# crisbodnar/text-to-image

Measured on AMD Instinct MI355X. Metric: images/sec (G+D step) at 64x64 batch=64, higher is better.
Workload: dtype f32; 1 GPU; wgancls 64x64 batch=64/GPU fp32, synthetic images + random 1024-d text embeddings, D step (+kt) then G step, Adam(b1=0,b2=0.9); global_batch=64, parallelism=dp1, launch=hipGraph replay (1 graph/iteration)

## Files before the change

### include/t2i_hip.h

```cpp
#ifndef T2I_HIP_H
#define T2I_HIP_H

#include <stddef.h>
#include <stdint.h>

#ifdef __cplusplus
extern "C" {
#endif

#define T2I_OK 0
#define T2I_ERR_INVALID (-1)
#define T2I_ERR_WORKSPACE (-2)
#define T2I_ERR_LAUNCH (-3)

#define T2I_ACT_NONE 0
#define T2I_ACT_LRELU 1
#define T2I_ACT_RELU 2
#define T2I_ACT_TANH 3

typedef void* t2i_stream_t;

enum { T2I_DT_F32 = 0, T2I_DT_BF16 = 1 };

typedef struct t2i_conv_desc {
// ... 79 lines not shown
               t2i_stream_t stream);

size_t t2i_bn_bwd_fused_workspace_bytes(int64_t rows, int32_t C);
int t2i_bn_bwd_fused(const void* dy, const void* y, const void* x, const float* mean, const float* rstd, const float* gamma, int64_t rows,
                     int32_t C, int act, float alpha, void* gmask, void* dx, void* dx_h, float* dgamma, float* dbeta, int accumulate, void* ws,
                     size_t ws_bytes, int32_t dtype , t2i_stream_t stream);

size_t t2i_bn_grouped_workspace_bytes(int64_t rows_per_group, int32_t C, int32_t groups);
int t2i_bn_train_fwd_grouped(const void* x, int64_t rows_per_group, int32_t C, int32_t groups, const float* gamma, const float* beta, float eps,
                             float decay, float* mean, float* rstd, float* scale, float* shift, float* moving_mean, float* moving_var, int act,
                             float alpha, void* y, void* y_h, const float* tile_sum, const float* tile_m2, int32_t tile_chunks, int32_t tile_rows,
                             int32_t moving_updates, int32_t moving_groups, void* ws, size_t ws_bytes, int32_t dtype, t2i_stream_t stream);
int t2i_bn_bwd_grouped(const void* dy, const void* y, const void* x, const float* mean, const float* rstd, const float* gamma, int64_t rows_per_group,
                       int32_t C, int32_t groups, int act, float alpha, void* gmask, void* dx, void* dx_h, float* dgamma, float* dbeta, int accumulate,
                       void* ws, size_t ws_bytes, int32_t dtype, t2i_stream_t stream);

int t2i_act_fwd(const void* x, int64_t n, int act, float alpha, void* y, void* y_h, int32_t dtype, t2i_stream_t stream);
int t2i_act_bwd(const void* dy, const void* y, int64_t n, int act, float alpha, void* dx, void* dx_h, int32_t dtype, t2i_stream_t stream);
int t2i_act_bwd_colsum(const void* dy, const void* y, const void* x2, const float* center, int64_t rows, int32_t C, int act,
                       float alpha, void* dx, void* dx_h, float* colsum, float* colsum_x2, int accumulate, void* ws, size_t ws_bytes,
                       int32_t dtype, t2i_stream_t stream);
int t2i_add_act(const void* a, const void* b, int64_t n, int act, float alpha, void* y, void* y_h, int32_t dtype, t2i_stream_t stream);
int t2i_axpby(const void* a, float alpha, const void* b, float beta, int64_t n, void* y, int32_t dtype, t2i_stream_t stream);
int t2i_interp(const float* eps, const float* g, const float* x, int32_t B, int64_t per_sample, float* xhat,
               t2i_stream_t stream);
int t2i_concat_tile_fwd(const void* feat, const void* emb, int32_t B, int32_t P, int32_t Cf, int32_t Ce,
                        void* out, int32_t dtype, t2i_stream_t stream);
int t2i_concat_tile_bwd(const void* dout, int32_t B, int32_t P, int32_t Cf, int32_t Ce, void* dfeat, void* demb,
                        int32_t dtype, t2i_stream_t stream);
int t2i_nchw_to_nhwc(const void* x, int32_t B, int32_t C, int32_t HW, void* y, int32_t dtype, t2i_stream_t stream);
// ... 189 lines not shown
```

### text-to-image_amd/_lib.py

```python
import ctypes
import os

import torch

_HERE = os.path.dirname(os.path.abspath(__file__))
LIB_PATH = os.environ.get('T2I_HIP_LIB', os.path.join(_HERE, 'lib', 'libt2i_hip.so'))


class ConvDesc(ctypes.Structure):
    _fields_ = [(n, ctypes.c_int32) for n in
                ('B', 'H', 'W', 'Cin', 'Ho', 'Wo', 'Cout', 'KH', 'KW', 'SH', 'SW', 'pad_t', 'pad_l', 'math')]


class ConvOpts(ctypes.Structure):
    _fields_ = [('a_image', ctypes.c_void_p), ('b_image', ctypes.c_void_p), ('out_image', ctypes.c_void_p), ('xform', ctypes.c_void_p),
                ('xform_bytes', ctypes.c_size_t), ('xform_mode', ctypes.c_int32), ('out_image_written', ctypes.c_int32),
                ('xform_kept', ctypes.c_int32), ('in_dtype', ctypes.c_int32), ('out_dtype', ctypes.c_int32), ('xform_valid_rows', ctypes.c_int32), ('xform_plane_rows', ctypes.c_int32), ('reserved', ctypes.c_int32)]


class ImageDesc(ctypes.Structure):
    _fields_ = [('offset', ctypes.c_int64)] + [(n, ctypes.c_int32) for n in
                                               ('height', 'width', 'channels', 'y1', 'y2', 'x1', 'x2', 'reserved')]


# ... 32 lines not shown
    't2i_interp': (ctypes.c_int, [_p, _p, _p, _i32, _i64, _p, _p]),
    't2i_concat_tile_fwd': (ctypes.c_int, [_p, _p, _i32, _i32, _i32, _i32, _p, _i32, _p]),
    't2i_concat_tile_bwd': (ctypes.c_int, [_p, _i32, _i32, _i32, _i32, _p, _p, _i32, _p]),
    't2i_nchw_to_nhwc': (ctypes.c_int, [_p, _i32, _i32, _i32, _p, _i32, _p]),
    't2i_nhwc_to_nchw': (ctypes.c_int, [_p, _i32, _i32, _i32, _p, _i32, _p]),
    't2i_gp_slopes': (ctypes.c_int, [_p, _i32, _i64, _p, _i32, _p]),
    't2i_row_scale': (ctypes.c_int, [_p, _p, _i32, _i64, _p, _i32, _p]),
    't2i_row_scale_div': (ctypes.c_int, [_p, _p, _p, _i32, _i64, _p, _i32, _p]),
    't2i_adam_tf': (ctypes.c_int, [_p, _p, _p, _p, _i64, _f, _p, _f, _f, _f, _f, _p]),
    't2i_adam_tf_ema': (ctypes.c_int, [_p, _p, _p, _p, _p, _i64, _f, _p, _f, _f, _f, _f, _f, _p, _p]),
    't2i_adam_tf_slots': (ctypes.c_int, [_p, _p, _p, _p, _p, _i64, _p, _p, _i32, _f, _p, _f, _f, _f, _f, _f, _p, _p]),
    't2i_wgan_d_head': (ctypes.c_int, [_p, _p, _p, _p, _i32, _f, _p, _p, _p, _p, _p]),
    't2i_bn_grouped_workspace_bytes': (_sz, [_i64, _i32, _i32]),
    't2i_bn_train_fwd_grouped': (ctypes.c_int, [_p, _i64, _i32, _i32, _p, _p, _f, _f, _p, _p, _p, _p, _p, _p, ctypes.c_int, _f, _p, _p, _p, _p, _i32, _i32, _i32, _i32, _p, _sz, _i32, _p]),
    't2i_bn_bwd_grouped': (ctypes.c_int, [_p, _p, _p, _p, _p, _p, _i64, _i32, _i32, ctypes.c_int, _f, _p, _p, _p, _p, _p, ctypes.c_int, _p, _sz, _i32, _p]),
    't2i_sigmoid_ce_head': (ctypes.c_int, [_p, _p, _p, _f, _f, _f, _f, _f, _f, _i32, _p, _p, _p, _p, _p, _p, _p, _p]),
    't2i_ca_kl_fwd': (ctypes.c_int, [_p, _p, _p, _i64, _p, _p, _p]),
    't2i_ca_kl_bwd': (ctypes.c_int, [_p, _p, _p, _p, _p, _i64, _p, _p, _p]),
    't2i_lerp_dev': (ctypes.c_int, [_p, _p, _p, _i32, _i64, _p, _p]),
    't2i_conv2d_algo': (ctypes.c_int, [_p, _i32]),
    't2i_stat': (ctypes.c_longlong, [ctypes.c_char_p]),
    't2i_conv2d_bwd_pair': (ctypes.c_int, [_dp, ctypes.c_int, _p, _p, _p, _op, _p, _p, _p, ctypes.c_int, _op, _p, _sz, _p, _sz, _p]),
    't2i_filter_cache_attach': (ctypes.c_int, [_p, _sz]),
    't2i_filter_cache_enable': (ctypes.c_int, [ctypes.c_int]),
    't2i_tuning_set': (ctypes.c_int, [ctypes.c_char_p, ctypes.c_double]),
    't2i_kt_sgd': (ctypes.c_int, [_p, _p, _f, _f, _p]),
    't2i_zero_ranges': (ctypes.c_int, [_p, _p, _i32, _p]),
    't2i_trunc_normal': (ctypes.c_int, [_p, _i64, ctypes.c_uint64, ctypes.c_uint64, _f, _f, _f, _f, _p]),
    't2i_filter_cache_invalidate': (None, [_p, ctypes.c_size_t]),
    't2i_filter_cache_bytes': (ctypes.c_size_t, []),
# ... 102 lines not shown
```

### text-to-image_amd/autograd.py

```python
import contextlib
import weakref

import torch
from torch.autograd import Function
from torch.autograd.function import once_differentiable

from . import kernels as K

_INPUTS_ONLY = [False]

SINKS = {}
NOTIFY = [None]


def register_sink(param, slot, first_touch=None):
    SINKS[param.data_ptr()] = (weakref.ref(param), slot, first_touch)


def sink_accumulate(ptr):
    e = SINKS.get(ptr)
    if e is None or e[2] is None:
        return True
    return not e[2]()

# ... 105 lines not shown
        ctx.set_materialize_grads(False)
        return K.act_bwd(_c(gy), y, act, alpha)

    @staticmethod
    def backward(ctx, gg):
        if gg is None:
            return None, None, None, None
        (y,) = ctx.saved_tensors
        return ActBwdFn.apply(gg, y, ctx.act, ctx.alpha), None, None, None


def _act_bwd(gy, y, act, alpha):
    return ActBwdFn.apply(gy, y, act, alpha) if act != K.ACT_NONE else _c(gy)


class ColSumFn(Function):

    @staticmethod
    def forward(ctx, a):
        ctx.shape, ctx.dtype = a.shape, a.dtype
        return K.col_reduce(_c(a))[0]

    @staticmethod
    def backward(ctx, g):
        return g.to(ctx.dtype).expand(ctx.shape)


class Conv2dFn(Function):

    @staticmethod
# ... 23 lines not shown


def conv2d_backward(x, w, y, gy, geom_b, act, alpha, has_bias, bias_ref, need, xform=None, xform_plane_rows=0):
    params = not _INPUTS_ONLY[0]
    want_b = has_bias and need[2] and params
    gb = None
    bsink = _sink_of(bias_ref) if want_b else None
    if (want_b and act != K.ACT_NONE and not torch.is_grad_enabled() and gy.shape[-1] % 4 == 0):
        gpre, gb = K.act_bwd_colsum(_c(gy), y, act, alpha, out=bsink)
        if bsink is not None:
            gb = None
            _notify(bias_ref)
    else:
        gpre = _act_bwd(gy, y, act, alpha)
        if want_b and bsink is not None:
            K.col_reduce(_c(gpre), out=bsink)
            _notify(bias_ref)
        elif want_b:
            gb = ColSumFn.apply(gpre)
    if need[0] and need[1] and params and _pair_ok(gpre, x, w):
        gx = K.conv_bwd_pair(K.PAIR_BWD_DATA, _c(gpre), w, _c(x), _c(gpre), geom_b[0], geom_b[1], sink_at(w.data_ptr()), out_dtype=x.dtype,
                             accumulate=sink_accumulate(w.data_ptr()))
        _notify(w)
        return gx, None, gb
    gx = ConvBwdDataFn.apply(gpre, w, None, geom_b, K.ACT_NONE, 0.0, x.dtype) if need[0] else None
    gw = _filter_grad(x, gpre, geom_b, w, xform, xform_plane_rows) if (need[1] and params) else None
    return gx, gw, gb


class ConvBwdDataFn(Function):

    @staticmethod
    def forward(ctx, dy, w, b, geom, act, alpha, out_dtype=None):
        d, ws = geom
# ... 18 lines not shown
def bwd_data_backward(dy, w, out, gg, geom_b, act, alpha, has_bias, bias_ref, need):
    gpre = _act_bwd(gg, out, act, alpha)
    params = not _INPUTS_ONLY[0]
    if need[0] and need[1] and params and _pair_ok(gpre, dy, w):
        g_dy = K.conv_bwd_pair(K.PAIR_FWD, _c(gpre), w, _c(gpre), _c(dy), geom_b[0], geom_b[1], sink_at(w.data_ptr()), out_dtype=dy.dtype,
                               accumulate=sink_accumulate(w.data_ptr()))
        _notify(w)
        g_w = None
    else:
        g_dy = Conv2dFn.apply(gpre, w, None, geom_b, K.ACT_NONE, 0.0, False, dy.dtype) if need[0] else None
        g_w = _filter_grad(gpre, dy, geom_b, w) if (need[1] and params) else None
    g_b = None
    if has_bias and need[2] and params:
        bsink = _sink_of(bias_ref)
        if bsink is not None:
            K.col_reduce(_c(gpre), out=bsink)
            _notify(bias_ref)
        else:
            g_b = ColSumFn.apply(gpre)
    return g_dy, g_w, g_b


class ConvBwdFilterFn(Function):

    @staticmethod
    def forward(ctx, x, dy, geom):
        d, ws = geom
        x, dy = _c(x), _c(dy)
        ctx.save_for_backward(x, dy)
        ctx.geom = geom
        return K.conv_bwd_filter(x, dy, d, ws)

    @staticmethod
    def backward(ctx, ggw):
# ... 112 lines not shown
        if gy is None:
            return (None,) * 10
        x, gamma, mean, rstd, y = ctx.saved_tensors
        gy = _c(gy)
        fused = gy.shape[-1] % 4 == 0 and all(t.data_ptr() % 16 == 0 for t in (gy, x, mean))
        if not fused:
            if ctx.act != K.ACT_NONE:
                gy = K.act_bwd(gy, y, ctx.act, ctx.alpha)
            sum_dy, sum_dy_x = K.col_reduce(gy, x, True, center=mean)
        want_g, want_b = ctx.needs_input_grad[1], ctx.needs_input_grad[2]
        gsink = _sink_of(ctx.gamma_ref) if want_g else None
        bsink = _sink_of(ctx.beta_ref) if want_b else None
        sunk = gsink is not None and bsink is not None
        if fused:
            dx, dgamma, dbeta = K.bn_bwd_grouped(gy, y if ctx.act != K.ACT_NONE else None, x, mean, rstd, gamma, 1, ctx.act, ctx.alpha,
                                                 dgamma_out=gsink if sunk else None, dbeta_out=bsink if sunk else None)
        else:
            dx, dgamma, dbeta = K.bn_bwd(gy, x, mean, rstd, gamma, sum_dy, sum_dy_x, dgamma_out=gsink if sunk else None,
                                         dbeta_out=bsink if sunk else None)
        if sunk:
            _notify(ctx.gamma_ref); _notify(ctx.beta_ref)
            return dx, None, None, None, None, None, None, None, None, None
        return dx, (dgamma if want_g else None), (dbeta if want_b else None), None, None, None, None, None, None, None


class BatchNormTrainGroupedFn(Function):

    @staticmethod
    def _fast(x, groups):
        b = x.shape[0] // groups
        return x.shape[-1] % 4 == 0 and x.data_ptr() % 16 == 0 and (x[:b].numel() * x.element_size()) % 16 == 0
# ... 472 lines not shown
```

### text-to-image_amd/csrc/t2i_aux.hip

```cpp
#include <hip/hip_runtime.h>
#include <stdlib.h>
#include <stdint.h>

#include <type_traits>

#include "t2i_internal.h"

namespace t2i {

static inline int ew_blocks(size_t n_items) {
  size_t b = (n_items + 255) / 256;
  if (b > 2048) b = 2048;
  if (b < 1) b = 1;
  return (int)b;
}

__device__ __forceinline__ float vadd(float a, float b) { return a + b; }
__device__ __forceinline__ float4 vadd(float4 a, float4 b) { return make_float4(a.x + b.x, a.y + b.y, a.z + b.z, a.w + b.w); }
__device__ __forceinline__ float vscale(float a, float s) { return a * s; }
__device__ __forceinline__ float4 vscale(float4 a, float s) { return make_float4(a.x * s, a.y * s, a.z * s, a.w * s); }

__device__ __forceinline__ float vsplat(float s, float) { return s; }
__device__ __forceinline__ float4 vsplat(float s, float4) { return make_float4(s, s, s, s); }

// ... 1013 lines not shown
  const int64_t rbeg = (int64_t)g_own * rows_g + (int64_t)j * rpb;
  int64_t rend = rbeg + rpb;
  if (rend > (int64_t)(g_own + 1) * rows_g) rend = (int64_t)(g_own + 1) * rows_g;
#pragma unroll 4
  for (int64_t r = rbeg + ty; r < rend; r += 16) {
    const size_t e4 = (size_t)(r * C + c) >> 2;
    float4 v = ld4<H>(x, e4);
    v.x = apply_act(v.x * sc.x + sh.x, act, alpha);
    v.y = apply_act(v.y * sc.y + sh.y, act, alpha);
    v.z = apply_act(v.z * sc.z + sh.z, act, alpha);
    v.w = apply_act(v.w * sc.w + sh.w, act, alpha);
    st4(y, yh, e4, v);
  }
}

template <bool HD, bool HX>
__global__ __launch_bounds__(256) void bn_bwd_apply_fused(const float* __restrict__ part0, const float* __restrict__ part1, int nchunks,
                                                          int64_t rows_g, int C, const float* __restrict__ mean, const float* __restrict__ rstd,
                                                          const float* __restrict__ gamma, float* __restrict__ dgamma, float* __restrict__ dbeta,
                                                          int accumulate, int groups, int64_t rpb, int nb_g, const void* __restrict__ gv,
                                                          const void* __restrict__ xv, float* __restrict__ dx, uint2* __restrict__ dxh) {
  __shared__ float4 red[16][16], red1[16][16];
  __shared__ float4 s_a[16], s_b[16], s_e[16];
  const int tx = threadIdx.x & 15, ty = threadIdx.x >> 4;
  const int c = blockIdx.x * 64 + tx * 4;
  const bool col_ok = c < C;
  const int g_own = blockIdx.y / nb_g, j = blockIdx.y - g_own * nb_g;
  const bool scribe = blockIdx.y == 0;
  const float n = (float)rows_g;
  float tg[4] = {0.f, 0.f, 0.f, 0.f}, tb[4] = {0.f, 0.f, 0.f, 0.f};
  for (int g = scribe ? 0 : g_own; g < (scribe ? groups : g_own + 1); ++g) {
    float4 a0 = make_float4(0.f, 0.f, 0.f, 0.f), a1 = make_float4(0.f, 0.f, 0.f, 0.f);
    if (col_ok) {
      for (int k = ty; k < nchunks; k += 16) {
        const size_t kk = (size_t)g * nchunks + k;
        const float4 v = *reinterpret_cast<const float4*>(part0 + kk * C + c);
        const float4 w = *reinterpret_cast<const float4*>(part1 + kk * C + c);
        a0.x += v.x; a0.y += v.y; a0.z += v.z; a0.w += v.w;
        a1.x += w.x; a1.y += w.y; a1.z += w.z; a1.w += w.w;
      }
    }
    __syncthreads();
    red[ty][tx] = a0;
    red1[ty][tx] = a1;
    __syncthreads();
    if (ty == 0 && col_ok) {
// ... 20 lines not shown
      }
      if (g == g_own) {
        s_a[tx] = make_float4(ka[0], ka[1], ka[2], ka[3]); s_b[tx] = make_float4(kb[0], kb[1], kb[2], kb[3]);
        s_e[tx] = make_float4(ke[0], ke[1], ke[2], ke[3]);
      }
    }
  }
  if (scribe && ty == 0 && col_ok) {
#pragma unroll
    for (int e = 0; e < 4; ++e) {
      dgamma[c + e] = accumulate ? dgamma[c + e] + tg[e] : tg[e];
      dbeta[c + e] = accumulate ? dbeta[c + e] + tb[e] : tb[e];
    }
  }
  __syncthreads();
  if (!col_ok) return;
  const float4 a = s_a[tx], b = s_b[tx], e = s_e[tx];
  const int64_t rbeg = (int64_t)g_own * rows_g + (int64_t)j * rpb;
  int64_t rend = rbeg + rpb;
  if (rend > (int64_t)(g_own + 1) * rows_g) rend = (int64_t)(g_own + 1) * rows_g;
#pragma unroll 4
  for (int64_t r = rbeg + ty; r < rend; r += 16) {
    const size_t e4 = (size_t)(r * C + c) >> 2;
    const float4 d = ld4<HD>(gv, e4);
    const float4 v = ld4<HX>(xv, e4);
    float4 o;
    o.x = a.x * d.x + b.x * v.x + e.x;
    o.y = a.y * d.y + b.y * v.y + e.y;
    o.z = a.z * d.z + b.z * v.z + e.z;
    o.w = a.w * d.w + b.w * v.w + e.w;
    st4(dx, dxh, e4, o);
  }
}

static void bn_fuse_rows(int64_t rows_g, int ct, int groups, int64_t* rpb, int* nb_g) {
  int64_t want = 1024 / ((int64_t)ct * groups);
  if (want < 1) want = 1;
  const int64_t maxb = (rows_g + 15) / 16;
  if (want > maxb) want = maxb;
  *rpb = (rows_g + want - 1) / want;
  *nb_g = (int)((rows_g + *rpb - 1) / *rpb);
}

static void bn_group_plan(int64_t rows_g, int C, int groups, int* ct, int* ncg, int64_t* rpc) {
  col_reduce_plan(rows_g, C, ct, ncg, rpc);
  const int cap = tuning().colred_cap / groups > 0 ? tuning().colred_cap / groups : 1;
  if (*ncg > cap) {
    *rpc = (rows_g + cap - 1) / cap;
    *ncg = (int)((rows_g + *rpc - 1) / *rpc);
  }
}

size_t bn_grouped_ws(int64_t rows_g, int C, int groups) {
  int ct, ncg; int64_t rpc;
  bn_group_plan(rows_g, C, groups, &ct, &ncg, &rpc);
  return ((size_t)groups * ncg * C * 2 + (size_t)groups * 3 * C) * sizeof(float);
}

hipError_t bn_fwd_grouped_launch(const void* x, int64_t rows_g, int C, int groups, const float* gamma, const float* beta, float eps, float decay,
                                 float* mean, float* rstd, float* scale, float* shift, float* mm, float* mv, int act, float alpha, float* y,
                                 void* y_h, void* ws, hipStream_t stream, bool x_bf16, const float* tile_sum, const float* tile_m2, int tile_chunks,
                                 int tile_rows, int moving_updates, int moving_groups) {
  int ct, ncg; int64_t rpc;
  bn_group_plan(rows_g, C, groups, &ct, &ncg, &rpc);
  const float* part0 = tile_sum;
// ... 29 lines not shown
#define T2I_BNS(TL, HH) hipLaunchKernelGGL((bn_stats_stage2_v4<TL, HH>), dim3((C + 15) / 16), dim3(256), 0, stream, part0, part1, x, ncg, rows_g, rpc, C, \
                                           (float*)nullptr, (float*)nullptr, fin, groups)
  if (tiles) { if (x_bf16) T2I_BNS(true, true); else T2I_BNS(true, false); }
  else { if (x_bf16) T2I_BNS(false, true); else T2I_BNS(false, false); }
#undef T2I_BNS
  const size_t n = (size_t)rows * C, pg4 = ((size_t)rows_g * C) >> 2;
  if (x_bf16)
    hipLaunchKernelGGL((bn_apply_kernel<true, true>), dim3(ew_blocks(n >> 2)), dim3(256), 0, stream, x, scale, shift, n, C, act, alpha, y, yh, pg4);
  else
    hipLaunchKernelGGL((bn_apply_kernel<true, false>), dim3(ew_blocks(n >> 2)), dim3(256), 0, stream, x, scale, shift, n, C, act, alpha, y, yh, pg4);
  return hipGetLastError();
}

hipError_t bn_bwd_grouped_launch(const void* dy, const void* y, const void* x, const float* mean, const float* rstd, const float* gamma,
                                 int64_t rows_g, int C, int groups, int act, float alpha, void* gmask, float* dx, float* dgamma, float* dbeta,
                                 int accumulate, void* ws, hipStream_t stream, void* dx_h, bool in_bf16) {
  int ct, ncg; int64_t rpc;
  bn_group_plan(rows_g, C, groups, &ct, &ncg, &rpc);
  const int64_t rows = rows_g * groups;
  float* part = reinterpret_cast<float*>(ws);
  float* part1 = part + (size_t)groups * ncg * C;
  float* coef = part1 + (size_t)groups * ncg * C;
  const void* g = dy;
  const dim3 grid(ct, groups * ncg);
  if (y) {
    if (in_bf16)
      hipLaunchKernelGGL((act_bwd_colsum_stage1<true, true>), grid, dim3(256), 0, stream, dy, y, x, mean, rows, C, rpc, act, alpha,
                         (float*)nullptr, part, part1, reinterpret_cast<unsigned short*>(gmask), rows_g, ncg);
    else
      hipLaunchKernelGGL((act_bwd_colsum_stage1<true, false>), grid, dim3(256), 0, stream, dy, y, x, mean, rows, C, rpc, act, alpha,
                         reinterpret_cast<float*>(gmask), part, part1, (unsigned short*)nullptr, rows_g, ncg);
    g = gmask;
  } else if (in_bf16) {
    hipLaunchKernelGGL((col_reduce_stage1_v4<true, true, true>), grid, dim3(256), 0, stream, dy, x, rows, C, rpc, part, part1, 0, mean, rows_g, ncg);
  } else {
    hipLaunchKernelGGL((col_reduce_stage1_v4<true, true, false>), grid, dim3(256), 0, stream, dy, x, rows, C, rpc, part, part1, 0, mean, rows_g, ncg);
  }
  if (tuning().bn_fuse && ncg <= BN_FUSE_MAX_CHUNKS) {
    int64_t rpb; int nb_g;
    bn_fuse_rows(rows_g, ct, groups, &rpb, &nb_g);
    const dim3 grid2(ct, groups * nb_g);
    if (in_bf16)
      hipLaunchKernelGGL((bn_bwd_apply_fused<true, true>), grid2, dim3(256), 0, stream, part, part1, ncg, rows_g, C, mean, rstd, gamma, dgamma, dbeta,
                         accumulate, groups, rpb, nb_g, g, x, dx, reinterpret_cast<uint2*>(dx_h));
    else
      hipLaunchKernelGGL((bn_bwd_apply_fused<false, false>), grid2, dim3(256), 0, stream, part, part1, ncg, rows_g, C, mean, rstd, gamma, dgamma, dbeta,
                         accumulate, groups, rpb, nb_g, g, x, dx, reinterpret_cast<uint2*>(dx_h));
    return hipGetLastError();
  }
  float* k_dy = coef; float* k_x = coef + C; float* k_0 = coef + 2 * (size_t)C;
  hipLaunchKernelGGL(bn_bwd_stage2_coef_v4, dim3(ct), dim3(256), 0, stream, part, part1, ncg, C, mean, rstd, gamma, (float)rows_g, dgamma, dbeta,
                     k_dy, k_x, k_0, accumulate, groups);
  const size_t n = (size_t)rows * C, pg4 = ((size_t)rows_g * C) >> 2;
  if (in_bf16)
    hipLaunchKernelGGL((bn_bwd_apply_kernel<true, true, true>), dim3(ew_blocks(n >> 2)), dim3(256), 0, stream, g, x, k_dy, k_x, k_0, n, C, dx,
                       reinterpret_cast<uint2*>(dx_h), pg4);
  else
    hipLaunchKernelGGL((bn_bwd_apply_kernel<true, false, false>), dim3(ew_blocks(n >> 2)), dim3(256), 0, stream, g, x, k_dy, k_x, k_0, n, C, dx,
                       reinterpret_cast<uint2*>(dx_h), pg4);
  return hipGetLastError();
}

hipError_t ew_launch(int op, const void* a, const void* b, size_t n_flag, int act, float alpha, float beta, float* y,
                     hipStream_t stream, void* y_h, bool in_bf16) {
  uint2* yh = reinterpret_cast<uint2*>(y_h);
  const bool al = (n_flag >> 63) == 0;
  const size_t n = n_flag & ~(1ull << 63);
  const size_t n4 = al ? (n >> 2) : 0;
  dim3 g(ew_blocks(al ? ((n + 3) >> 2) : n)), blk(256);
// ... 731 lines not shown
```

### text-to-image_amd/csrc/t2i_capi.hip

```cpp
#include <hip/hip_runtime.h>
#include <atomic>
#include <initializer_list>
#include <stdarg.h>
#include <stdio.h>
#include <stdlib.h>
#include <string.h>

#include "t2i_internal.h"

namespace t2i {

static thread_local char g_err[512] = "";

void set_error(const char* fmt, ...) {
  va_list ap;
  va_start(ap, fmt);
  vsnprintf(g_err, sizeof(g_err), fmt, ap);
  va_end(ap);
}

size_t col_reduce_ws(int64_t rows, int C);
hipError_t col_reduce_launch(const void*, const void*, const float*, int64_t, int, float*, float*, int, void*, hipStream_t, bool in_bf16 = false);
hipError_t bn_stats_launch(const void*, int64_t, int, float*, float*, const float*, const float*, float, float, float*, float*, float*,
                           float*, float*, float*, void*, hipStream_t, bool x_bf16 = false);
hipError_t bn_stats_tiles_launch(const float*, const float*, int, int, int64_t, int, float*, float*, const float*, const float*, float, float,
                                 float*, float*, float*, float*, float*, float*, hipStream_t);
hipError_t bn_bwd_fused_launch(const void*, const void*, const void*, const float*, const float*, const float*, int64_t, int, int, float,
                               void*, float*, float*, float*, int, void*, hipStream_t, void* dx_h, bool in_bf16);
hipError_t bn_finalize_launch(const float*, const float*, int64_t, int, const float*, const float*, float, float, float*,
                              float*, float*, float*, float*, float*, hipStream_t);
hipError_t bn_apply_launch(const void*, const float*, const float*, int64_t, int, int, float, float*, hipStream_t, void* y_h, bool x_bf16);
hipError_t bn_infer_launch(const void* x, const float* gamma, const float* beta, const float* mm, const float* mv, float eps, int64_t rows,
                           int C, int act, float alpha, const void* residual, int res_act, float res_alpha, void* y, hipStream_t stream,
                           bool vec, bool x_bf16);
size_t bn_grouped_ws(int64_t rows_g, int C, int groups);
hipError_t bn_fwd_grouped_launch(const void*, int64_t, int, int, const float*, const float*, float, float, float*, float*, float*, float*, float*, float*,
                                 int, float, float*, void*, void*, hipStream_t, bool, const float*, const float*, int, int, int, int);
hipError_t bn_bwd_grouped_launch(const void*, const void*, const void*, const float*, const float*, const float*, int64_t, int, int, int, float, void*,
                                 float*, float*, float*, int, void*, hipStream_t, void*, bool);
hipError_t bn_bwd_launch(const float*, const float*, const float*, const float*, const float*, const float*, const float*,
                         int64_t, int, float*, float*, float*, float*, int, hipStream_t);
hipError_t ew_launch(int, const void*, const void*, size_t, int, float, float, float*, hipStream_t, void* y_h, bool in_bf16);
hipError_t interp_launch(const float*, const float*, const float*, int, int64_t, float*, hipStream_t);
hipError_t concat_tile_fwd_launch(const void*, const void*, int, int, int, int, void*, hipStream_t, bool bf16);
hipError_t concat_tile_bwd_launch(const void*, int, int, int, int, void*, void*, hipStream_t, bool bf16);
hipError_t transpose_launch(const void*, int, int, int, void*, hipStream_t, bool bf16);
hipError_t gp_slopes_launch(const void*, int, int64_t, float*, hipStream_t, bool bf16);
hipError_t row_scale_launch(const void*, const float*, int, int64_t, void*, hipStream_t, bool bf16 = false, const float* den = nullptr);
hipError_t crop_flip_normalize_launch(const uint8_t*, int, const int32_t*, const int32_t*, const int32_t*, const int32_t*, int, int, float*, hipStream_t);
hipError_t gather_mean_launch(const float*, int, int, const int32_t*, const int32_t*, int, int, float*, hipStream_t);
size_t nearest_images_ws(int Q, int64_t N);
hipError_t nearest_images_launch(const uint8_t*, int, int, const int32_t*, const int32_t*, const int32_t*, const float*, int, int, float,
                                 float, int32_t*, double*, void*, hipStream_t);
size_t resample_bilinear_ws(int B, int Hi, int Wo);
// ... 1212 lines not shown
    set_error("t2i_bn_train_fwd_grouped: bad argument (C %% 4 == 0 required)");
    return T2I_ERR_INVALID;
  }
  if (!(aligned16(x) && aligned16(y) && aligned16(scale) && aligned16(shift) && aligned16(y_h))) {
    set_error("t2i_bn_train_fwd_grouped: tensors must be 16-byte aligned");
    return T2I_ERR_INVALID;
  }
  if (!ws || ws_bytes < bn_grouped_ws(rows_per_group, C, groups) || !aligned16(ws)) { set_error("t2i_bn_train_fwd_grouped: workspace too small"); return T2I_ERR_WORKSPACE; }
  if (int rc = h_contract(dtype, true, C, y_h, "t2i_bn_train_fwd_grouped")) return rc;
  const bool h = dtype == T2I_DT_BF16;
  return check(bn_fwd_grouped_launch(x, rows_per_group, C, groups, gamma, beta, eps, decay, mean, rstd, scale, shift, moving_mean, moving_var, act, alpha,
                                     h ? nullptr : reinterpret_cast<float*>(y), h ? y : y_h, ws, (hipStream_t)stream, h, tile_sum, tile_m2, tile_chunks, tile_rows, moving_updates, moving_groups),
               "t2i_bn_train_fwd_grouped");
}

int t2i_bn_bwd_grouped(const void* dy, const void* y, const void* x, const float* mean, const float* rstd, const float* gamma, int64_t rows_per_group,
                       int32_t C, int32_t groups, int act, float alpha, void* gmask, void* dx, void* dx_h, float* dgamma, float* dbeta, int accumulate,
                       void* ws, size_t ws_bytes, int32_t dtype, t2i_stream_t stream) {
  if (!dy || !x || !mean || !rstd || !gamma || !dx || !dgamma || !dbeta || rows_per_group <= 0 || C <= 0 || (C & 3) || groups <= 0 || (y && !gmask)) {
    set_error("t2i_bn_bwd_grouped: bad argument (C %% 4 == 0 required; gmask needed with an activation)");
    return T2I_ERR_INVALID;
  }
  {
    const int64_t lim = ((int64_t)1 << 30) - 16;
    if (rows_per_group > lim / C || rows_per_group * C > lim / groups) {
      set_error("t2i_bn_bwd_grouped: rows_per_group * groups * C exceeds 2^30 - 16 elements");
      return T2I_ERR_INVALID;
    }
  }
  if (!(aligned16(dy) && aligned16(x) && aligned16(dx) && aligned16(mean) && aligned16(dx_h) && (!y || (aligned16(y) && aligned16(gmask))))) {
    set_error("t2i_bn_bwd_grouped: tensors must be 16-byte aligned");
    return T2I_ERR_INVALID;
  }
  if (!ws || ws_bytes < bn_grouped_ws(rows_per_group, C, groups) || !aligned16(ws)) { set_error("t2i_bn_bwd_grouped: workspace too small"); return T2I_ERR_WORKSPACE; }
  if (int rc = h_contract(dtype, true, C, dx_h, "t2i_bn_bwd_grouped")) return rc;
  const bool h = dtype == T2I_DT_BF16;
  return check(bn_bwd_grouped_launch(dy, y, x, mean, rstd, gamma, rows_per_group, C, groups, act, alpha, gmask, h ? nullptr : reinterpret_cast<float*>(dx),
                                     dgamma, dbeta, accumulate ? 1 : 0, ws, (hipStream_t)stream, h ? dx : dx_h, h), "t2i_bn_bwd_grouped");
}

int t2i_bn_bwd(const float* dy, const float* x, const float* mean, const float* rstd, const float* gamma,
               const float* sum_dy, const float* sum_dy_x, int64_t rows, int32_t C, float* dx, float* dgamma, float* dbeta,
               int accumulate, void* ws, size_t ws_bytes, t2i_stream_t stream) {
  if (!dy || !x || !mean || !rstd || !gamma || !sum_dy || !sum_dy_x || !dx || !dgamma || !dbeta || rows <= 0 || C <= 0) {
    set_error("t2i_bn_bwd: bad argument");
    return T2I_ERR_INVALID;
  }
  if (!ws || ws_bytes < (size_t)3 * C * sizeof(float) || !aligned16(ws)) { set_error("t2i_bn_bwd: workspace too small"); return T2I_ERR_WORKSPACE; }
  const bool al = aligned16(dy) && aligned16(x) && aligned16(dx);
  return check(bn_bwd_launch(dy, x, mean, rstd, gamma, sum_dy, sum_dy_x, rows, al ? C : -C, dx, dgamma, dbeta,
                             reinterpret_cast<float*>(ws), accumulate ? 1 : 0, (hipStream_t)stream), "t2i_bn_bwd");
}

// ... 869 lines not shown
```

### text-to-image_amd/kernels.py

```python
import contextlib
import ctypes
import os

import numpy as np
import torch

from ._lib import DT_BF16, DT_F32, XFORM_HAVE, XFORM_KEEP, ConvDesc, ConvOpts, ImageDesc, check, lib

ACT_NONE, ACT_LRELU, ACT_RELU, ACT_TANH = 0, 1, 2, 3

_DRY = [False]


@contextlib.contextmanager
def dry_run():
    prev = _DRY[0]
    _DRY[0] = True
    try:
        yield
    finally:
        _DRY[0] = prev


def is_dry():
# ... 703 lines not shown
            hit = None
        tsum = tm2 = None
        tchunks = trows = 0
        if hit is not None:
            part, chunks, trows, _ = hit
            tsum, tm2, tchunks = ctypes.c_void_p(part.data_ptr()), ctypes.c_void_p(part.data_ptr() + chunks * C * 4), chunks // groups
        wsp, wsn = _ws_args(x, int(lib.t2i_bn_grouped_workspace_bytes(rows_g, C, groups)))
        twin = _twin_for(y, x)
        check(lib.t2i_bn_train_fwd_grouped(_ptr(x), rows_g, C, groups, _ptr(_chk(gamma)), _ptr(_chk(beta)), eps, decay, _ptr(stat[0]), _ptr(stat[1]),
                                           _ptr(stat[2]), _ptr(stat[3]), _ptr(moving_mean), _ptr(moving_var), act, alpha, _ptr(y), _ptr(twin),
                                           tsum, tm2, tchunks, trows, int(moving_updates), int(moving_groups), wsp, wsn, _dt(x), _stream()), 't2i_bn_train_fwd_grouped')
        _twin_keep(y, twin)
    return y, stat[0], stat[1]


def bn_bwd_grouped(dy, y, x, mean, rstd, gamma, groups, act, alpha=0.2, dgamma_out=None, dbeta_out=None):
    _chk(dy, 'dy'); _chk(x, 'x')
    C = x.shape[-1]
    rows_g = x.numel() // C // groups
    dx = torch.empty_like(x)
    gmask = torch.empty_like(x) if y is not None else None
    acc = dgamma_out is not None
    assert acc == (dbeta_out is not None)
    dgamma = dgamma_out if acc else torch.empty(C, dtype=torch.float32, device=x.device)
    dbeta = dbeta_out if acc else torch.empty(C, dtype=torch.float32, device=x.device)
    if _live(x):
        wsp, wsn = _ws_args(x, int(lib.t2i_bn_grouped_workspace_bytes(rows_g, C, groups)))
        twin = _twin_for(dx)
        check(lib.t2i_bn_bwd_grouped(_ptr(dy), _ptr(_chk(y, 'y') if y is not None else None), _ptr(x), _ptr(mean), _ptr(rstd), _ptr(_chk(gamma)),
                                     rows_g, C, groups, act, alpha, _ptr(gmask), _ptr(dx), _ptr(twin), _ptr(dgamma), _ptr(dbeta), 1 if acc else 0,
                                     wsp, wsn, _same_dt(dy, y, x), _stream()), 't2i_bn_bwd_grouped')
        _twin_keep(dx, twin)
    return dx, dgamma, dbeta


_bn_apply_one = bn_apply


def bn_bwd(dy, x, mean, rstd, gamma, sum_dy, sum_dy_x, dgamma_out=None, dbeta_out=None):
    _chk(dy, 'dy'); _chk(x, 'x')
    C = x.shape[-1]
    dx = torch.empty_like(x)
    acc = dgamma_out is not None
    assert acc == (dbeta_out is not None)
    dgamma = dgamma_out if acc else torch.empty(C, dtype=torch.float32, device=x.device)
    dbeta = dbeta_out if acc else torch.empty(C, dtype=torch.float32, device=x.device)
    if _live(x):
        wsp, wsn = _ws_args(x, 3 * C * 4)
# ... 54 lines not shown
    _chk(a, 'a'); _chk(b, 'b')
    assert a.shape == b.shape
    y = torch.empty_like(a)
    if _live(a):
        twin = _twin_for(y, a, b)
        check(lib.t2i_add_act(_ptr(a), _ptr(b), a.numel(), act, alpha, _ptr(y), _ptr(twin), _same_dt(a, b), _stream()), 't2i_add_act')
        _twin_keep(y, twin)
    return y


def _drop_image(t):
    if t is not None:
        h = _image_holder(t)
        if getattr(h, '_t2i_h', None) is not None:
            h._t2i_h = None


def axpby(a, alpha, b=None, beta=0.0, out=None):
    _chk(a, 'a')
    y = torch.empty_like(a) if out is None else out
    _drop_image(out)
    if _live(a):
        check(lib.t2i_axpby(_ptr(a), alpha, _ptr(_chk(b, 'b') if b is not None else None), beta, a.numel(), _ptr(y),
                            _same_dt(a, b, y), _stream()), 't2i_axpby')
    return y


def interp(eps, g, x, out=None):
    _chk(g, 'g', f32=True); _chk(x, 'x', f32=True)
    eps = _chk(eps.reshape(-1), 'eps', f32=True)
# ... 1034 lines not shown
```

### text-to-image_amd/stacked.py

```python
import torch
from torch.autograd import Function

from . import autograd as A
from . import kernels as K

_FIRST = [0]


class first_order_pass(object):

    def __init__(self, rows):
        self.rows = int(rows)

    def __enter__(self):
        self.prev, _FIRST[0] = _FIRST[0], self.rows

    def __exit__(self, *a):
        _FIRST[0] = self.prev


class Stacked(object):
    __slots__ = ('main', 'hat')

    def __init__(self, main, hat):
# ... 355 lines not shown
    def backward(ctx, gym, gyh):
        if gym is None and gyh is None:
            return (None,) * 13
        x4, gamma, mean, rstd, y4 = ctx.saved_tensors
        R, gm = ctx.R, ctx.gm
        want_g, want_b = ctx.needs_input_grad[2], ctx.needs_input_grad[3]
        gsink = A._sink_of(ctx.gamma_ref) if want_g else None
        bsink = A._sink_of(ctx.beta_ref) if want_b else None
        sunk = gsink is not None and bsink is not None
        outs = [None, None]
        dgamma = dbeta = None
        for i, (g, sl, gs) in enumerate(((gym, slice(0, R), slice(0, gm)), (gyh, slice(R, x4.shape[0]), slice(gm, ctx.groups)))):
            if g is None:
                continue
            dx, dg, db = K.bn_bwd_grouped(_c(g), y4[sl] if y4 is not None else None, x4[sl], mean[gs], rstd[gs], gamma, gs.stop - gs.start, ctx.act,
                                          ctx.alpha, dgamma_out=gsink if sunk else None, dbeta_out=bsink if sunk else None)
            outs[i] = dx
            if not sunk:
                dgamma = dg if dgamma is None else dgamma + dg
                dbeta = db if dbeta is None else dbeta + db
        if sunk:
            A._notify(ctx.gamma_ref); A._notify(ctx.beta_ref)
            dgamma = dbeta = None
        return (outs[0], outs[1], dgamma if want_g else None, dbeta if want_b else None) + (None,) * 9


def batch_norm_ok(x, groups=2):
    m, h = x.main, x.hat
    rows = m.shape[0] + h.shape[0]
    if rows % groups or m.shape[0] % (rows // groups) or not (m.is_contiguous() and h.is_contiguous()):
        return False
# ... 68 lines not shown
```

Baseline: 5250 images/sec.

## Fuse conv bias-gradient column partials into batchnorm backward apply kernel

The batchnorm backward apply kernel now also writes per-block column sums of the dx it produces into a side buffer. That buffer is attached to the dx tensor, so the next conv layer's bias-gradient reduction can finish from the partials without rereading the full gradient. This removes one full read pass over the gradient for each such conv bias. In exchange the fused path uses the coarser chunk grid instead of the wider grid2 row split, adds a partials buffer allocation, and relies on version and pointer checks to keep the cached partials valid.

```diff
diff --git a/include/t2i_hip.h b/include/t2i_hip.h
--- a/include/t2i_hip.h
+++ b/include/t2i_hip.h
@@ -117,6 +117,11 @@
 int t2i_bn_bwd_grouped(const void* dy, const void* y, const void* x, const float* mean, const float* rstd, const float* gamma, int64_t rows_per_group,
                        int32_t C, int32_t groups, int act, float alpha, void* gmask, void* dx, void* dx_h, float* dgamma, float* dbeta, int accumulate,
                        void* ws, size_t ws_bytes, int32_t dtype, t2i_stream_t stream);
+size_t t2i_bn_bias_partials_bytes(int64_t rows_per_group, int32_t C, int32_t groups);
+int t2i_bn_bwd_grouped_bias(const void* dy, const void* y, const void* x, const float* mean, const float* rstd, const float* gamma, int64_t rows_per_group,
+                            int32_t C, int32_t groups, int act, float alpha, void* gmask, void* dx, void* dx_h, float* dgamma, float* dbeta,
+                            int accumulate, void* ws, size_t ws_bytes, int32_t dtype, float* bias_part, size_t bias_part_bytes, int32_t* bias_chunks,
+                            t2i_stream_t stream);
 
 int t2i_act_fwd(const void* x, int64_t n, int act, float alpha, void* y, void* y_h, int32_t dtype, t2i_stream_t stream);
 int t2i_act_bwd(const void* dy, const void* y, int64_t n, int act, float alpha, void* dx, void* dx_h, int32_t dtype, t2i_stream_t stream);
diff --git a/text-to-image_amd/_lib.py b/text-to-image_amd/_lib.py
--- a/text-to-image_amd/_lib.py
+++ b/text-to-image_amd/_lib.py
@@ -70,6 +70,9 @@
     't2i_bn_grouped_workspace_bytes': (_sz, [_i64, _i32, _i32]),
     't2i_bn_train_fwd_grouped': (ctypes.c_int, [_p, _i64, _i32, _i32, _p, _p, _f, _f, _p, _p, _p, _p, _p, _p, ctypes.c_int, _f, _p, _p, _p, _p, _i32, _i32, _i32, _i32, _p, _sz, _i32, _p]),
     't2i_bn_bwd_grouped': (ctypes.c_int, [_p, _p, _p, _p, _p, _p, _i64, _i32, _i32, ctypes.c_int, _f, _p, _p, _p, _p, _p, ctypes.c_int, _p, _sz, _i32, _p]),
+    't2i_bn_bias_partials_bytes': (_sz, [_i64, _i32, _i32]),
+    't2i_bn_bwd_grouped_bias': (ctypes.c_int, [_p, _p, _p, _p, _p, _p, _i64, _i32, _i32, ctypes.c_int, _f, _p, _p, _p, _p, _p, ctypes.c_int, _p, _sz, _i32,
+                                               _p, _sz, _p, _p]),
     't2i_sigmoid_ce_head': (ctypes.c_int, [_p, _p, _p, _f, _f, _f, _f, _f, _f, _i32, _p, _p, _p, _p, _p, _p, _p, _p]),
     't2i_ca_kl_fwd': (ctypes.c_int, [_p, _p, _p, _i64, _p, _p, _p]),
     't2i_ca_kl_bwd': (ctypes.c_int, [_p, _p, _p, _p, _p, _i64, _p, _p, _p]),
diff --git a/text-to-image_amd/autograd.py b/text-to-image_amd/autograd.py
--- a/text-to-image_amd/autograd.py
+++ b/text-to-image_amd/autograd.py
@@ -143,6 +143,11 @@
     return ActBwdFn.apply(gy, y, act, alpha) if act != K.ACT_NONE else _c(gy)
 
 
+def _bias_colsum(gpre, bsink):
+    if K.col_reduce_taken(gpre, out=bsink) is None:
+        K.col_reduce(_c(gpre), out=bsink)
+
+
 class ColSumFn(Function):
 
     @staticmethod
@@ -196,10 +201,12 @@
     else:
         gpre = _act_bwd(gy, y, act, alpha)
         if want_b and bsink is not None:
-            K.col_reduce(_c(gpre), out=bsink)
+            _bias_colsum(gpre, bsink)
             _notify(bias_ref)
         elif want_b:
-            gb = ColSumFn.apply(gpre)
+            gb = K.col_reduce_taken(gpre)
+            if gb is None:
+                gb = ColSumFn.apply(gpre)
     if need[0] and need[1] and params and _pair_ok(gpre, x, w):
         gx = K.conv_bwd_pair(K.PAIR_BWD_DATA, _c(gpre), w, _c(x), _c(gpre), geom_b[0], geom_b[1], sink_at(w.data_ptr()), out_dtype=x.dtype,
                              accumulate=sink_accumulate(w.data_ptr()))
@@ -248,10 +255,12 @@
     if has_bias and need[2] and params:
         bsink = _sink_of(bias_ref)
         if bsink is not None:
-            K.col_reduce(_c(gpre), out=bsink)
+            _bias_colsum(gpre, bsink)
             _notify(bias_ref)
         else:
-            g_b = ColSumFn.apply(gpre)
+            g_b = K.col_reduce_taken(gpre)
+            if g_b is None:
+                g_b = ColSumFn.apply(gpre)
     return g_dy, g_w, g_b
 
 
@@ -394,7 +403,7 @@
         sunk = gsink is not None and bsink is not None
         if fused:
             dx, dgamma, dbeta = K.bn_bwd_grouped(gy, y if ctx.act != K.ACT_NONE else None, x, mean, rstd, gamma, 1, ctx.act, ctx.alpha,
-                                                 dgamma_out=gsink if sunk else None, dbeta_out=bsink if sunk else None)
+                                                 dgamma_out=gsink if sunk else None, dbeta_out=bsink if sunk else None, bias_partials=True)
         else:
             dx, dgamma, dbeta = K.bn_bwd(gy, x, mean, rstd, gamma, sum_dy, sum_dy_x, dgamma_out=gsink if sunk else None,
                                          dbeta_out=bsink if sunk else None)
diff --git a/text-to-image_amd/csrc/t2i_aux.hip b/text-to-image_amd/csrc/t2i_aux.hip
--- a/text-to-image_amd/csrc/t2i_aux.hip
+++ b/text-to-image_amd/csrc/t2i_aux.hip
@@ -1051,22 +1051,29 @@
   }
 }
 
-template <bool HD, bool HX>
+template <bool HD, bool HX, bool COEF = false, bool BP = false>
 __global__ __launch_bounds__(256) void bn_bwd_apply_fused(const float* __restrict__ part0, const float* __restrict__ part1, int nchunks,
                                                           int64_t rows_g, int C, const float* __restrict__ mean, const float* __restrict__ rstd,
                                                           const float* __restrict__ gamma, float* __restrict__ dgamma, float* __restrict__ dbeta,
                                                           int accumulate, int groups, int64_t rpb, int nb_g, const void* __restrict__ gv,
-                                                          const void* __restrict__ xv, float* __restrict__ dx, uint2* __restrict__ dxh) {
+                                                          const void* __restrict__ xv, float* __restrict__ dx, uint2* __restrict__ dxh,
+                                                          float* __restrict__ bpart = nullptr) {
   __shared__ float4 red[16][16], red1[16][16];
   __shared__ float4 s_a[16], s_b[16], s_e[16];
   const int tx = threadIdx.x & 15, ty = threadIdx.x >> 4;
   const int c = blockIdx.x * 64 + tx * 4;
   const bool col_ok = c < C;
   const int g_own = blockIdx.y / nb_g, j = blockIdx.y - g_own * nb_g;
-  const bool scribe = blockIdx.y == 0;
+  const bool scribe = !COEF && blockIdx.y == 0;
   const float n = (float)rows_g;
   float tg[4] = {0.f, 0.f, 0.f, 0.f}, tb[4] = {0.f, 0.f, 0.f, 0.f};
-  for (int g = scribe ? 0 : g_own; g < (scribe ? groups : g_own + 1); ++g) {
+  if (COEF && ty == 0 && col_ok) {
+    const float* k = part0 + (size_t)g_own * 3 * C + c;
+    s_a[tx] = *reinterpret_cast<const float4*>(k);
+    s_b[tx] = *reinterpret_cast<const float4*>(k + C);
+    s_e[tx] = *reinterpret_cast<const float4*>(k + 2 * (size_t)C);
+  }
+  for (int g = scribe ? 0 : g_own; !COEF && g < (scribe ? groups : g_own + 1); ++g) {
     float4 a0 = make_float4(0.f, 0.f, 0.f, 0.f), a1 = make_float4(0.f, 0.f, 0.f, 0.f);
     if (col_ok) {
       for (int k = ty; k < nchunks; k += 16) {
@@ -1117,22 +1124,36 @@
     }
   }
   __syncthreads();
-  if (!col_ok) return;
-  const float4 a = s_a[tx], b = s_b[tx], e = s_e[tx];
-  const int64_t rbeg = (int64_t)g_own * rows_g + (int64_t)j * rpb;
-  int64_t rend = rbeg + rpb;
-  if (rend > (int64_t)(g_own + 1) * rows_g) rend = (int64_t)(g_own + 1) * rows_g;
+  if (!BP && !col_ok) return;
+  float4 acc = make_float4(0.f, 0.f, 0.f, 0.f);
+  if (col_ok) {
+    const float4 a = s_a[tx], b = s_b[tx], e = s_e[tx];
+    const int64_t rbeg = (int64_t)g_own * rows_g + (int64_t)j * rpb;
+    int64_t rend = rbeg + rpb;
+    if (rend > (int64_t)(g_own + 1) * rows_g) rend = (int64_t)(g_own + 1) * rows_g;
 #pragma unroll 4
-  for (int64_t r = rbeg + ty; r < rend; r += 16) {
-    const size_t e4 = (size_t)(r * C + c) >> 2;
-    const float4 d = ld4<HD>(gv, e4);
-    const float4 v = ld4<HX>(xv, e4);
-    float4 o;
-    o.x = a.x * d.x + b.x * v.x + e.x;
-    o.y = a.y * d.y + b.y * v.y + e.y;
-    o.z = a.z * d.z + b.z * v.z + e.z;
-    o.w = a.w * d.w + b.w * v.w + e.w;
-    st4(dx, dxh, e4, o);
+    for (int64_t r = rbeg + ty; r < rend; r += 16) {
+      const size_t e4 = (size_t)(r * C + c) >> 2;
+      const float4 d = ld4<HD>(gv, e4);
+      const float4 v = ld4<HX>(xv, e4);
+      float4 o;
+      o.x = a.x * d.x + b.x * v.x + e.x;
+      o.y = a.y * d.y + b.y * v.y + e.y;
+      o.z = a.z * d.z + b.z * v.z + e.z;
+      o.w = a.w * d.w + b.w * v.w + e.w;
+      st4(dx, dxh, e4, o);
+      if (BP) { acc.x += o.x; acc.y += o.y; acc.z += o.z; acc.w += o.w; }
+    }
+  }
+  if (BP) {
+    red[ty][tx] = acc;
+    __syncthreads();
+    if (ty == 0 && col_ok) {
+      float4 s0 = red[0][tx];
+#pragma unroll
+      for (int k = 1; k < 16; ++k) { const float4 v = red[k][tx]; s0.x += v.x; s0.y += v.y; s0.z += v.z; s0.w += v.w; }
+      *reinterpret_cast<float4*>(bpart + (size_t)blockIdx.y * C + c) = s0;
+    }
   }
 }
 
@@ -1152,6 +1173,12 @@
     *rpc = (rows_g + cap - 1) / cap;
     *ncg = (int)((rows_g + *rpc - 1) / *rpc);
   }
+}
+
+size_t bn_bias_partials_floats(int64_t rows_g, int C, int groups) {
+  int ct, ncg; int64_t rpc;
+  bn_group_plan(rows_g, C, groups, &ct, &ncg, &rpc);
+  return (size_t)groups * ncg * C;
 }
 
 size_t bn_grouped_ws(int64_t rows_g, int C, int groups) {
@@ -1211,13 +1238,15 @@
 
 hipError_t bn_bwd_grouped_launch(const void* dy, const void* y, const void* x, const float* mean, const float* rstd, const float* gamma,
                                  int64_t rows_g, int C, int groups, int act, float alpha, void* gmask, float* dx, float* dgamma, float* dbeta,
-                                 int accumulate, void* ws, hipStream_t stream, void* dx_h, bool in_bf16) {
+                                 int accumulate, void* ws, hipStream_t stream, void* dx_h, bool in_bf16, float* bpart, int* bchunks) {
   int ct, ncg; int64_t rpc;
   bn_group_plan(rows_g, C, groups, &ct, &ncg, &rpc);
   const int64_t rows = rows_g * groups;
   float* part = reinterpret_cast<float*>(ws);
   float* part1 = part + (size_t)groups * ncg * C;
   float* coef = part1 + (size_t)groups * ncg * C;
+  if (bchunks) *bchunks = 0;
+  if (in_bf16) bpart = nullptr;
   const void* g = dy;
   const dim3 grid(ct, groups * ncg);
   if (y) {
@@ -1237,7 +1266,11 @@
     int64_t rpb; int nb_g;
     bn_fuse_rows(rows_g, ct, groups, &rpb, &nb_g);
     const dim3 grid2(ct, groups * nb_g);
-    if (in_bf16)
+    if (bpart) {
+      hipLaunchKernelGGL((bn_bwd_apply_fused<false, false, false, true>), grid, dim3(256), 0, stream, part, part1, ncg, rows_g, C, mean, rstd, gamma,
+                         dgamma, dbeta, accumulate, groups, rpc, ncg, g, x, dx, reinterpret_cast<uint2*>(dx_h), bpart);
+      *bchunks = groups * ncg;
+    } else if (in_bf16)
       hipLaunchKernelGGL((bn_bwd_apply_fused<true, true>), grid2, dim3(256), 0, stream, part, part1, ncg, rows_g, C, mean, rstd, gamma, dgamma, dbeta,
                          accumulate, groups, rpb, nb_g, g, x, dx, reinterpret_cast<uint2*>(dx_h));
     else
@@ -1249,7 +1282,11 @@
   hipLaunchKernelGGL(bn_bwd_stage2_coef_v4, dim3(ct), dim3(256), 0, stream, part, part1, ncg, C, mean, rstd, gamma, (float)rows_g, dgamma, dbeta,
                      k_dy, k_x, k_0, accumulate, groups);
   const size_t n = (size_t)rows * C, pg4 = ((size_t)rows_g * C) >> 2;
-  if (in_bf16)
+  if (bpart) {
+    hipLaunchKernelGGL((bn_bwd_apply_fused<false, false, true, true>), grid, dim3(256), 0, stream, (const float*)coef, (const float*)nullptr, ncg, rows_g,
+                       C, mean, rstd, gamma, dgamma, dbeta, accumulate, groups, rpc, ncg, g, x, dx, reinterpret_cast<uint2*>(dx_h), bpart);
+    *bchunks = groups * ncg;
+  } else if (in_bf16)
     hipLaunchKernelGGL((bn_bwd_apply_kernel<true, true, true>), dim3(ew_blocks(n >> 2)), dim3(256), 0, stream, g, x, k_dy, k_x, k_0, n, C, dx,
                        reinterpret_cast<uint2*>(dx_h), pg4);
   else
diff --git a/text-to-image_amd/csrc/t2i_capi.hip b/text-to-image_amd/csrc/t2i_capi.hip
--- a/text-to-image_amd/csrc/t2i_capi.hip
+++ b/text-to-image_amd/csrc/t2i_capi.hip
@@ -37,7 +37,8 @@
 hipError_t bn_fwd_grouped_launch(const void*, int64_t, int, int, const float*, const float*, float, float, float*, float*, float*, float*, float*, float*,
                                  int, float, float*, void*, void*, hipStream_t, bool, const float*, const float*, int, int, int, int);
 hipError_t bn_bwd_grouped_launch(const void*, const void*, const void*, const float*, const float*, const float*, int64_t, int, int, int, float, void*,
-                                 float*, float*, float*, int, void*, hipStream_t, void*, bool);
+                                 float*, float*, float*, int, void*, hipStream_t, void*, bool, float* bpart, int* bchunks);
+size_t bn_bias_partials_floats(int64_t rows_g, int C, int groups);
 hipError_t bn_bwd_launch(const float*, const float*, const float*, const float*, const float*, const float*, const float*,
                          int64_t, int, float*, float*, float*, float*, int, hipStream_t);
 hipError_t ew_launch(int, const void*, const void*, size_t, int, float, float, float*, hipStream_t, void* y_h, bool in_bf16);
@@ -1280,9 +1281,9 @@
                "t2i_bn_train_fwd_grouped");
 }
 
-int t2i_bn_bwd_grouped(const void* dy, const void* y, const void* x, const float* mean, const float* rstd, const float* gamma, int64_t rows_per_group,
-                       int32_t C, int32_t groups, int act, float alpha, void* gmask, void* dx, void* dx_h, float* dgamma, float* dbeta, int accumulate,
-                       void* ws, size_t ws_bytes, int32_t dtype, t2i_stream_t stream) {
+static int bn_bwd_grouped_impl(const void* dy, const void* y, const void* x, const float* mean, const float* rstd, const float* gamma, int64_t rows_per_group,
+                               int32_t C, int32_t groups, int act, float alpha, void* gmask, void* dx, void* dx_h, float* dgamma, float* dbeta, int accumulate,
+                               void* ws, size_t ws_bytes, int32_t dtype, float* bias_part, int* bias_chunks, t2i_stream_t stream) {
   if (!dy || !x || !mean || !rstd || !gamma || !dx || !dgamma || !dbeta || rows_per_group <= 0 || C <= 0 || (C & 3) || groups <= 0 || (y && !gmask)) {
     set_error("t2i_bn_bwd_grouped: bad argument (C %% 4 == 0 required; gmask needed with an activation)");
     return T2I_ERR_INVALID;
@@ -1302,7 +1303,37 @@
   if (int rc = h_contract(dtype, true, C, dx_h, "t2i_bn_bwd_grouped")) return rc;
   const bool h = dtype == T2I_DT_BF16;
   return check(bn_bwd_grouped_launch(dy, y, x, mean, rstd, gamma, rows_per_group, C, groups, act, alpha, gmask, h ? nullptr : reinterpret_cast<float*>(dx),
-                                     dgamma, dbeta, accumulate ? 1 : 0, ws, (hipStream_t)stream, h ? dx : dx_h, h), "t2i_bn_bwd_grouped");
+                                     dgamma, dbeta, accumulate ? 1 : 0, ws, (hipStream_t)stream, h ? dx : dx_h, h, bias_part, bias_chunks), "t2i_bn_bwd_grouped");
+}
+
+int t2i_bn_bwd_grouped(const void* dy, const void* y, const void* x, const float* mean, const float* rstd, const float* gamma, int64_t rows_per_group,
+                       int32_t C, int32_t groups, int act, float alpha, void* gmask, void* dx, void* dx_h, float* dgamma, float* dbeta, int accumulate,
+                       void* ws, size_t ws_bytes, int32_t dtype, t2i_stream_t stream) {
+  return bn_bwd_grouped_impl(dy, y, x, mean, rstd, gamma, rows_per_group, C, groups, act, alpha, gmask, dx, dx_h, dgamma, dbeta, accumulate, ws, ws_bytes,
+                             dtype, nullptr, nullptr, stream);
+}
+
+size_t t2i_bn_bias_partials_bytes(int64_t rows_per_group, int32_t C, int32_t groups) {
+  if (rows_per_group <= 0 || C <= 0 || groups <= 0) return 0;
+  return bn_bias_partials_floats(rows_per_group, C, groups) * sizeof(float);
+}
+
+int t2i_bn_bwd_grouped_bias(const void* dy, const void* y, const void* x, const float* mean, const float* rstd, const float* gamma, int64_t rows_per_group,
+                            int32_t C, int32_t groups, int act, float alpha, void* gmask, void* dx, void* dx_h, float* dgamma, float* dbeta,
+                            int accumulate, void* ws, size_t ws_bytes, int32_t dtype, float* bias_part, size_t bias_part_bytes, int32_t* bias_chunks,
+                            t2i_stream_t stream) {
+  if (!bias_chunks) { set_error("t2i_bn_bwd_grouped_bias: bias_chunks is NULL"); return T2I_ERR_INVALID; }
+  *bias_chunks = 0;
+  if (!bias_part || !aligned16(bias_part)) { set_error("t2i_bn_bwd_grouped_bias: bias_part must be a 16-byte aligned buffer"); return T2I_ERR_INVALID; }
+  if (rows_per_group > 0 && C > 0 && groups > 0 && bias_part_bytes < t2i_bn_bias_partials_bytes(rows_per_group, C, groups)) {
+    set_error("t2i_bn_bwd_grouped_bias: bias_part is shorter than t2i_bn_bias_partials_bytes");
+    return T2I_ERR_INVALID;
+  }
+  int chunks = 0;
+  const int rc = bn_bwd_grouped_impl(dy, y, x, mean, rstd, gamma, rows_per_group, C, groups, act, alpha, gmask, dx, dx_h, dgamma, dbeta, accumulate, ws,
+                                     ws_bytes, dtype, bias_part, &chunks, stream);
+  if (rc == T2I_OK) *bias_chunks = chunks;
+  return rc;
 }
 
 int t2i_bn_bwd(const float* dy, const float* x, const float* mean, const float* rstd, const float* gamma,
diff --git a/text-to-image_amd/kernels.py b/text-to-image_amd/kernels.py
--- a/text-to-image_amd/kernels.py
+++ b/text-to-image_amd/kernels.py
@@ -741,7 +741,7 @@
     return y, stat[0], stat[1]
 
 
-def bn_bwd_grouped(dy, y, x, mean, rstd, gamma, groups, act, alpha=0.2, dgamma_out=None, dbeta_out=None):
+def bn_bwd_grouped(dy, y, x, mean, rstd, gamma, groups, act, alpha=0.2, dgamma_out=None, dbeta_out=None, bias_partials=False):
     _chk(dy, 'dy'); _chk(x, 'x')
     C = x.shape[-1]
     rows_g = x.numel() // C // groups
@@ -754,11 +754,40 @@
     if _live(x):
         wsp, wsn = _ws_args(x, int(lib.t2i_bn_grouped_workspace_bytes(rows_g, C, groups)))
         twin = _twin_for(dx)
-        check(lib.t2i_bn_bwd_grouped(_ptr(dy), _ptr(_chk(y, 'y') if y is not None else None), _ptr(x), _ptr(mean), _ptr(rstd), _ptr(_chk(gamma)),
-                                     rows_g, C, groups, act, alpha, _ptr(gmask), _ptr(dx), _ptr(twin), _ptr(dgamma), _ptr(dbeta), 1 if acc else 0,
-                                     wsp, wsn, _same_dt(dy, y, x), _stream()), 't2i_bn_bwd_grouped')
+        if bias_partials and dx.dtype == torch.float32:
+            nbytes = int(lib.t2i_bn_bias_partials_bytes(rows_g, C, groups))
+            part = torch.empty(nbytes // 4, dtype=torch.float32, device=x.device)
+            chunks = ctypes.c_int32(0)
+            check(lib.t2i_bn_bwd_grouped_bias(_ptr(dy), _ptr(_chk(y, 'y') if y is not None else None), _ptr(x), _ptr(mean), _ptr(rstd),
+                                              _ptr(_chk(gamma)), rows_g, C, groups, act, alpha, _ptr(gmask), _ptr(dx), _ptr(twin), _ptr(dgamma),
+                                              _ptr(dbeta), 1 if acc else 0, wsp, wsn, _same_dt(dy, y, x), _ptr(part), nbytes, ctypes.byref(chunks),
+                                              _stream()), 't2i_bn_bwd_grouped_bias')
+            if chunks.value > 0:
+                dx._t2i_bp = (part, int(chunks.value), dx._version, dx.data_ptr(), tuple(dx.shape))
+        else:
+            check(lib.t2i_bn_bwd_grouped(_ptr(dy), _ptr(_chk(y, 'y') if y is not None else None), _ptr(x), _ptr(mean), _ptr(rstd), _ptr(_chk(gamma)),
+                                         rows_g, C, groups, act, alpha, _ptr(gmask), _ptr(dx), _ptr(twin), _ptr(dgamma), _ptr(dbeta), 1 if acc else 0,
+                                         wsp, wsn, _same_dt(dy, y, x), _stream()), 't2i_bn_bwd_grouped')
         _twin_keep(dx, twin)
     return dx, dgamma, dbeta
+
+
+def col_reduce_taken(a, out=None):
+    h = _image_holder(a)
+    hit = getattr(h, '_t2i_bp', None)
+    if hit is None:
+        return None
+    part, chunks, version, ptr, shape = hit
+    if (h._version != version or h.data_ptr() != ptr or tuple(h.shape) != shape or a.data_ptr() != ptr or not a.is_contiguous()
+            or a.numel() != h.numel() or a.shape[-1] != shape[-1]):
+        return None
+    C = a.shape[-1]
+    if out is not None:
+        assert out.numel() == C
+        _drop_image(out)
+    out0 = out if out is not None else torch.empty(C, dtype=torch.float32, device=a.device)
+    check(lib.t2i_col_reduce_partials(_ptr(part), None, chunks, C, _ptr(out0), None, 1 if out is not None else 0, _stream()), 't2i_col_reduce_partials')
+    return out0
 
 
 _bn_apply_one = bn_apply
@@ -843,6 +872,9 @@
         h = _image_holder(t)
         if getattr(h, '_t2i_h', None) is not None:
             h._t2i_h = None
+        for o in (t, h):
+            if getattr(o, '_t2i_bp', None) is not None:
+                o._t2i_bp = None
 
 
 def axpby(a, alpha, b=None, beta=0.0, out=None):
diff --git a/text-to-image_amd/stacked.py b/text-to-image_amd/stacked.py
--- a/text-to-image_amd/stacked.py
+++ b/text-to-image_amd/stacked.py
@@ -393,7 +393,7 @@
             if g is None:
                 continue
             dx, dg, db = K.bn_bwd_grouped(_c(g), y4[sl] if y4 is not None else None, x4[sl], mean[gs], rstd[gs], gamma, gs.stop - gs.start, ctx.act,
-                                          ctx.alpha, dgamma_out=gsink if sunk else None, dbeta_out=bsink if sunk else None)
+                                          ctx.alpha, dgamma_out=gsink if sunk else None, dbeta_out=bsink if sunk else None, bias_partials=True)
             outs[i] = dx
             if not sunk:
                 dgamma = dg if dgamma is None else dgamma + dg
```

Result: no change. 5249 images/sec (-0.0%).
